# marcottelab/FluorosequencingImageAnalysis

Measured on AMD Instinct MI355X. Metric: psf_lm_fits_per_sec, higher is better.
Workload: dtype f64

## Files before the change

fluorosequencingimageanalysis_amd/csrc/fsq_fit_rounds.hip:

```cpp
#include <algorithm>
#include <atomic>
#include <cstdlib>

#include <mutex>
#include <new>
#include <type_traits>
#include <vector>

#include "fsq_common.h"
#include "fsq_lm_quad.h"
#include "fsq_evalguard.h"

namespace {

#define WAVE_SYNC() do { __builtin_amdgcn_fence(__ATOMIC_RELEASE, "wavefront"); __builtin_amdgcn_wave_barrier(); \
                         __builtin_amdgcn_fence(__ATOMIC_ACQUIRE, "wavefront"); } while (0)

#ifdef FSQ_DEBUG_HZ
__device__ unsigned long long g_hz[32];
#endif
#ifdef FSQ_PHASE_PROFILE
__device__ unsigned long long g_rphase[32];
#define RPH_DECL unsigned long long rph_t0 = clock64(), rph_acc[16] = {0,0,0,0,0,0,0,0,0,0,0,0,0,0,0,0};
#define RPH_MARK(k) { unsigned long long t_ = clock64(); rph_acc[k] += t_ - rph_t0; rph_t0 = t_; }
#define RPH_FLUSH(off) if (threadIdx.x == 0 && (blockIdx.x & 63) == 0) { for (int k_ = 0; k_ < 16; k_++) atomicAdd(&g_rphase[(off) + k_], rph_acc[k_]); }
#else
#define RPH_DECL
#define RPH_MARK(k)
#define RPH_FLUSH(off)
#endif

enum { CNT_A = 0, CNT_BLO = 1, CNT_BHI = 2, CNT_C1 = 3, CNT_C3 = 4, CNT_SET = 8 };
enum { Q_EPS = Q_WA3 };
enum { A_IDX = 0, A_X = 1, A_DIAG = 8, A_LLIM1 = 15, A_FNORM = 16, A_PAR = 17, A_DELTA = 18, A_XNORM = 19, A_ITER = 20,
       A_HDR = 21 , A_E = 21 , A_LEN = 46,
       B_GNORM = 21, B_IPVT = 22, B_QTF = 23, B_SDIAG = 30, B_R = 37, B_LEN = 65,
       C_PARL = 65, C_PARU = 66, C_FP = 67, C_LMIT = 68, C_LEN = 69 };

struct FitOut {
    double x[FSQ_NP];
    int status, niter, nfev, pad;
};
struct FitStat {
    double vmax, vmean;
};

struct Ctx {
    uint16_t* roi;
    int pix32;
    FitOut* out;
    FitStat* stat;
    long long cap;
    long long pool;
    int* err;
    int* slow_total;
    int* done;
    int tshift;
    int wave_prio;
    int force_redo;
    int force_slow_mod;
};

enum { G_KINIT_POS = 1, G_KINIT_SLOT = 2, G_KA_BLO = 3, G_KA_BHI = 4, G_KA_OVERLAP = 5, G_KA_SLOW = 6, G_KB_C1 = 7, G_KB_C3 = 8, G_KB_A = 9,
       G_KB_BLO = 10, G_KB_BHI = 11 };
FSQ_DEV long long fsq_guard(const Ctx& c, long long v, long long limit, int code)
{
    if ((unsigned long long)v < (unsigned long long)limit) return v;
    atomicMax(c.err, code);
    return 0;
}

FSQ_DEV int wave_reserve(int* counter, bool want)
{
    const unsigned long long m = __ballot(want);
    if (m == 0) return 0;
    const int lane = threadIdx.x & 63;
    const int leader = __ffsll((long long)m) - 1;
    int base = 0;
    if (lane == leader) base = atomicAdd(counter, __popcll(m));
    base = __shfl(base, leader);
    return base + __popcll(m & ((1ull << lane) - 1ull));
}

FSQ_DEV long long wave_reserve_checked(const Ctx& c, int* counter, bool want, long long limit, int code)
{
    const int at = wave_reserve(counter, want);
    return want ? fsq_guard(c, at, limit, code) : 0;
}

struct BatchArgs {
    const uint16_t* src; const int32_t* cand; int H, W; long long n; int from_image;
    int pix_fmt;
    long long base;
    int ticket;
    int no_queue;
};

FSQ_DEV void wave_mark_done(int* done, bool term, int ticket)
{
    unsigned long long m = __ballot(term);
    const int lane = threadIdx.x & 63;
    while (m) {
        const int leader = __ffsll((long long)m) - 1;
        const int t = __shfl(ticket, leader);
        const unsigned long long mm = __ballot(term && ticket == t);
        if (lane == leader) atomicAdd(done + t, __popcll(mm));
        m &= ~mm;
    }
}

#ifndef FSQ_NT
#define FSQ_NT 0
#endif
typedef unsigned fsq_u4v __attribute__((ext_vector_type(4)));
// ... 170 lines not shown
    double d = (S[0] + S[2]) + (S[1] + S[3]);
#pragma unroll
    for (int i = 16; i < 25; i++) { double v = QL(off, i); d = fsq_fma(v, v, d); }
    return d;
}

#define KA_ROWS(i) do { if (L == 8 && ((i) % 5) == 4) __builtin_amdgcn_sched_barrier(0); } while (0)
#define KA_EVAL_LOOP _Pragma("unroll EVAL_UNROLL")
#define KA_PIN(v) do { if (FAST) asm volatile("" : "+v"(v)); } while (0)
#ifdef FSQ_DEBUG_HZ
#define KA_HZ(code, cond) do { if (cond) { hz = true; if (FAST) atomicAdd(&g_hz[code], 1ull); } } while (0)
#else
#define KA_HZ(code, cond) do { if (cond) hz = true; } while (0)
#endif
template <bool FAST, int L, bool P32 = false>
__global__ void __launch_bounds__(64, (L == 8 ? 4 : 2)) kA_jacobian(Ctx c, const double* __restrict__ QA, const int* __restrict__ cntA_p,
                                                                    double* __restrict__ QB, int* __restrict__ cnt_cur,
                                                                    double* __restrict__ SQ, int* __restrict__ slow_cnt,
                                                                    int* __restrict__ next_counters)
{
    constexpr int G = 64 / L;
    constexpr int NC = 8 / L;
    constexpr int MPX = (FSQ_NPIX + L - 1) / L;
    constexpr int MREC = (A_HDR + L - 1) / L;
    constexpr bool EVAL_ALL = FAST && L == 4;
    constexpr int EVAL_UNROLL = EVAL_ALL ? MPX : 1;
    static_assert(fsq_llim(4, 0.) == FSQ_EG_MIN_SIGMA && fsq_llim(5, 0.) == FSQ_EG_MIN_SIGMA, "fsq_evalguard.h: sigma floor != the fit's lower limit");
    __shared__ double lds[Q_KA_END * G];
    const int lane = threadIdx.x, grp = lane / L, cl = lane % L, gbase = lane - cl;
    const int n7 = FSQ_NP;
    if (c.wave_prio) __builtin_amdgcn_s_setprio(3);
    const int cntA = FAST ? *cntA_p : *slow_cnt;
    if (!FAST && blockIdx.x == 0 && threadIdx.x == 0 && cntA > 0) atomicAdd(c.slow_total, cntA);
    if (FAST && blockIdx.x == 0 && threadIdx.x < CNT_SET) next_counters[threadIdx.x] = 0;
    double col[NC][FSQ_NPIX];
    RPH_DECL
    const long long cap = c.cap;
    const int stride = gridDim.x * G;
    int base = blockIdx.x * G;
    if (base >= cntA) return;
    do {
        RPH_MARK(0)
        const bool active = (base + grp) < cntA;
        const NtQ qa = ntq(QA + (active ? base + grp : 0));
        double rec[MREC];
#pragma unroll
        for (int m = 0; m < MREC; m++) { const int f = cl + L * m; rec[m] = (active && f < A_HDR) ? (double)qa[f * cap] : 0.0; }
        bool hz = false, qhz = false;
        int emin = 0;
        int tag, niter, nfev, hist;
        unpack2(__shfl(rec[A_IDX / L], gbase + A_IDX % L), &tag, &hist);
        unpack2(__shfl(rec[A_ITER / L], gbase + A_ITER % L), &niter, &nfev);
        const bool b_hi = hist > 1;
        const int at_lo = wave_reserve(cnt_cur + CNT_BLO, active && cl == 0 && !b_hi);
        const int at_hi = wave_reserve(cnt_cur + CNT_BHI, active && cl == 0 && b_hi);
#ifdef FSQ_EXPERIMENT_EXTRA_ATOMICS_KA
        {
            int sink = 0;
            for (int x = 0; x < FSQ_EXPERIMENT_EXTRA_ATOMICS_KA; x++) sink += wave_reserve(cnt_cur + 5 + (x & 1), active && cl == 0);
            if (sink == 0x7fffffff) atomicMax(c.err, 99);
        }
#endif
        if (active && cl == 0) {
            if (!b_hi) fsq_guard(c, at_lo, cap, G_KA_BLO); else fsq_guard(c, at_hi, cap, G_KA_BHI);
            if ((long long)at_lo + (long long)at_hi + 2 > cap && (at_lo > 0 || at_hi > 0)) {
                const int nlo = b_hi ? cnt_cur[CNT_BLO] : at_lo + 1, nhi = b_hi ? at_hi + 1 : cnt_cur[CNT_BHI];
                if ((long long)nlo + nhi > cap) atomicMax(c.err, (int)G_KA_OVERLAP);
            }
        }
        const long long at = __shfl((active && cl == 0) ? (int)fsq_guard(c, b_hi ? (long long)(cap - 1) - at_hi : (long long)at_lo, cap, b_hi ? G_KA_BHI : G_KA_BLO) : 0, gbase);
        const int idx = tag_slot(c, tag);
        const bool fresh = active && (nfev == 0);
        double llim1 = 0., fnorm = 0., xnorm = 0., delta = 0., par_in = 0.;
        unsigned ipvt = 0x76543210u;
        int status = 0;
        double gnorm = 0.;
        uint4 roi = make_uint4(0u, 0u, 0u, 0u);
        uint4 roi_hi = make_uint4(0u, 0u, 0u, 0u);
        double ev[MPX];
#pragma unroll
        for (int m = 0; m < MPX; m++) ev[m] = 0.0;
        if (active) {
            if (P32) {
                static_assert(!P32 || L == 4, "32-bit pixels: the four-lane Jacobian round only");
                const uint32_t* r32 = (const uint32_t*)c.roi + (size_t)idx * 32 + cl * 8;
                roi = nt_ld4(r32); roi_hi = nt_ld4(r32 + 4);
            } else if (L == 4) roi = nt_ld4(c.roi + (size_t)idx * 32 + cl * 8);
            else {
                const unsigned long long w8 = fsq_bits(nt_ld((const double*)(c.roi + (size_t)idx * 32 + cl * 4)));
                roi.x = (unsigned)w8; roi.y = (unsigned)(w8 >> 32);
            }
            if (!fresh) {
#pragma unroll
                for (int m = 0; m < MPX; m++) { const int k = cl + L * m; if (k < FSQ_NPIX) ev[m] = qa[(A_E + k) * cap]; }
            }
#pragma unroll
            for (int m = 0; m < MREC; m++) {
                const int f = cl + L * m;
                if (f >= 1 && f <= 19) QL(Q_X, f - 1) = rec[m];
            }
        }
        WAVE_SYNC();
        RPH_MARK(1)
// ... 507 lines not shown
                    while (rem >= 7 - i) { rem -= 7 - i; i++; }
                    qb[(B_R + e) * cap] = QRG(i, i + rem);
                }
                for (int k = cl; k < FSQ_NP; k += L) {
                    qb[(A_X + k) * cap] = QL(Q_X, k);
                    qb[(A_DIAG + k) * cap] = QL(Q_DIAG, k);
                    qb[(B_QTF + k) * cap] = QL(Q_QTF, k);
                    qb[(B_SDIAG + k) * cap] = 0.;
                }
                if (cl == 0) {
                    qb[A_IDX * cap] = pack2(tag, hist);
                    qb[A_LLIM1 * cap] = llim1; qb[A_FNORM * cap] = fnorm; qb[A_PAR * cap] = par_in; qb[A_DELTA * cap] = delta;
                    qb[A_XNORM * cap] = xnorm; qb[A_ITER * cap] = pack2(niter, nfev);
                    qb[B_GNORM * cap] = gnorm; qb[B_IPVT * cap] = pack2((int)ipvt, 0);
                }
            } else if (active && cl == 0) qb[A_IDX * cap] = pack2(-1, 0);
        }
        RPH_MARK(6)
        base += stride;
    } while (!FAST && base < cntA);
    RPH_FLUSH(16)
}
#undef QRG
#undef REFL
#undef KA_ROWS
#undef KA_PIN
#undef KA_EVAL_LOOP
#undef KA_HZ
#pragma pop_macro("QL")

#ifndef FSQ_KA_LANES_DEFAULT
#define FSQ_KA_LANES_DEFAULT 4
#endif
#ifndef FSQ_LMPAR_FIRST
#define FSQ_LMPAR_FIRST 5
#endif
#ifndef FSQ_LMPAR_LO
#define FSQ_LMPAR_LO 1
#endif
#ifndef FSQ_KB_WAVES
#define FSQ_KB_WAVES 2
#endif
FSQ_DEV int kb_res_slot(int i) { return i < 14 ? i : i + 7; }

template <bool FAST>
FSQ_DEV bool kb_trial_gauss(const double* p, double* myscr)
{
    bool bad = false;
    double s, c;
    fsq_sincos(FSQ_PI_180 * p[6], &s, &c);
    const double rcen_x = p[3] * c - p[2] * s;
    const double rcen_y = p[3] * s + p[2] * c;
    const FsqDivisor k4 = fsq_divisor(p[4]), k5 = fsq_divisor(p[5]);
    if (FAST)
        bad = !fsq_divisor_in_range(p[4]) || !fsq_divisor_in_range(p[5]) || !(__builtin_fabs(p[2]) <= 0x1p100) ||
              !(__builtin_fabs(p[3]) <= 0x1p100) || !fsq_evalguard_ok(c, s, rcen_x, rcen_y, p[4], p[5]);
#pragma unroll 1
    for (int xi = 0; xi < 5; xi++) {
        const double x = (double)xi;
#pragma unroll
        for (int yi = 0; yi < 5; yi++) {
            const double y = (double)yi;
            const double xp = x * c - y * s;
            const double yp = x * s + y * c;
            const double nu = rcen_x - xp, nv = rcen_y - yp;
            myscr[kb_res_slot(xi * 5 + yi) * 64] = ka_gauss<FAST>(nu, nv, k4, k5);
        }
    }
    return bad;
}

FSQ_DEV double kb_late_load(const NtRef r) { asm volatile("" ::: "memory"); return (double)r; }

struct KbLimits { int lim[4]; };
template <bool ALIASED, bool P32 = false>
__global__ void __launch_bounds__(64, FSQ_KB_WAVES) kB_step(Ctx c, const double* __restrict__ QB, const double* __restrict__ QC,
                                                  const int* __restrict__ cnt_cur,
                                                  double* __restrict__ QA_next, double* __restrict__ QB_next, double* __restrict__ QC_next,
                                                  int* __restrict__ cnt_next, KbLimits lims)
{
    __shared__ double scr[32 * 64];
    if (c.wave_prio) __builtin_amdgcn_s_setprio(3);
    const int lane = threadIdx.x;
    const long long cap = c.cap;
    double* myscr = scr + lane;
    RPH_DECL
    {
        int b = blockIdx.x, seg, cnt;
        const int n_lo = cnt_cur[CNT_BLO], n_hi = cnt_cur[CNT_BHI], n_c1 = cnt_cur[CNT_C1], n_c3 = cnt_cur[CNT_C3];
        if (b < (n_c3 + 63) / 64) { seg = 3; cnt = n_c3; }
        else if ((b -= (n_c3 + 63) / 64) < (n_hi + 63) / 64) { seg = 1; cnt = n_hi; }
        else if ((b -= (n_hi + 63) / 64) < (n_c1 + 63) / 64) { seg = 2; cnt = n_c1; }
        else if ((b -= (n_c1 + 63) / 64) < (n_lo + 63) / 64) { seg = 0; cnt = n_lo; }
        else return;
        const bool resume = seg >= 2;
        const int lm_limit = lims.lim[seg];
        const int base = b * 64;
        RPH_MARK(0)
        bool live = (base + lane) < cnt;
        const int p_in = live ? (base + lane) : base;
        const NtQ qb = ntq((resume ? QC : QB) + ((seg & 1) ? cap - 1 - p_in : p_in));
        int tag = 0, dummy, niter = 1, nfev = 1, ipvt_i = 0x76543210;
        {
            int t;
            unpack2(qb[A_IDX * cap], &t, &dummy);
            if (t == -1) live = false;
            if (live) tag = t;
        }
        QuadLm q;
        double xq[FSQ_NP];
        double llim1 = 0., fnorm = 1., par = 0., delta = 1., xnorm = 1., fnorm1;
        if (live) {
            unpack2(qb[A_ITER * cap], &niter, &nfev);
            unpack2(qb[B_IPVT * cap], &ipvt_i, &dummy);
#pragma unroll
            for (int i = 0; i < FSQ_NP; i++)
#pragma unroll
                for (int k = 0; k < FSQ_NP; k++) q.r[i][k] = (k >= i) ? (double)qb[(B_R + rpk(i, k)) * cap] : 0.0;
#pragma unroll
            for (int k = 0; k < FSQ_NP; k++) {
                q.qtf[k] = qb[(B_QTF + k) * cap]; q.dg[k] = qb[(A_DIAG + k) * cap]; q.sdiag[k] = qb[(B_SDIAG + k) * cap];
                xq[k] = qb[(A_X + k) * cap];
            }
            llim1 = qb[A_LLIM1 * cap];
            fnorm = qb[A_FNORM * cap]; par = qb[A_PAR * cap]; delta = qb[A_DELTA * cap]; xnorm = qb[A_XNORM * cap];
        } else {
            const double x0[FSQ_NP] = {100., 1000., 2.5, 2.5, 1., 1., 0.};
#pragma unroll
            for (int i = 0; i < FSQ_NP; i++)
#pragma unroll
                for (int k = 0; k < FSQ_NP; k++) q.r[i][k] = (k == i) ? 1.0 : 0.0;
#pragma unroll
            for (int k = 0; k < FSQ_NP; k++) { q.qtf[k] = 0.; q.dg[k] = 1.; q.sdiag[k] = 0.; xq[k] = x0[k]; }
        }
        const unsigned ipvt = (unsigned)ipvt_i;
#define KB_GNORM() kb_late_load(qb[B_GNORM * cap])
#pragma unroll
        for (int k = 0; k < FSQ_NP; k++) myscr[k * 64] = q.dg[k];
#pragma unroll
        for (int j = 0; j < FSQ_NP; j++) q.dgp[j] = myscr[nib_get(ipvt, j) * 64];

        RPH_MARK(1)
        int lm_hist = 0;
        {
            QuadLmparSt st;
            if (!resume) quadlm_lmpar_begin<ALIASED, 64>(q, myscr, ipvt, delta, par, st);
            else if (live) {
                int it, dm;
                unpack2(qb[C_LMIT * cap], &it, &dm);
                st.par = par; st.parl = qb[C_PARL * cap]; st.paru = qb[C_PARU * cap]; st.fp = qb[C_FP * cap];
                st.iter = it; st.done = false;
            } else { st.par = 0.; st.parl = 0.; st.paru = 0.; st.fp = 0.; st.iter = 10; st.done = true; }
            RPH_MARK(7)
            quadlm_lmpar_run<ALIASED, 64>(q, myscr, ipvt, delta, st, lm_limit);
            par = st.par;
            lm_hist = st.iter;
            {
                const bool park = live && !st.done;
                const bool to_c1 = (st.iter < lims.lim[2]);
                const int at1 = (int)wave_reserve_checked(c, cnt_next + CNT_C1, park && to_c1, cap, G_KB_C1);
                const int at3 = (int)wave_reserve_checked(c, cnt_next + CNT_C3, park && !to_c1, cap, G_KB_C3);
                if (park) {
                    const NtQ qn = ntq(QC_next + (to_c1 ? (long long)at1 : cap - 1 - at3));
                    qn[A_IDX * cap] = pack2(tag, 0);
#pragma unroll
                    for (int k = 0; k < FSQ_NP; k++) {
                        qn[(A_X + k) * cap] = xq[k]; qn[(A_DIAG + k) * cap] = q.dg[k];
                        qn[(B_QTF + k) * cap] = q.qtf[k]; qn[(B_SDIAG + k) * cap] = q.sdiag[k];
                    }
                    qn[A_LLIM1 * cap] = llim1; qn[A_FNORM * cap] = fnorm; qn[A_PAR * cap] = par; qn[A_DELTA * cap] = delta;
                    qn[A_XNORM * cap] = xnorm; qn[A_ITER * cap] = pack2(niter, nfev);
                    qn[B_GNORM * cap] = KB_GNORM(); qn[B_IPVT * cap] = pack2((int)ipvt, 0);
#pragma unroll
                    for (int i = 0; i < FSQ_NP; i++)
#pragma unroll
                        for (int k = i; k < FSQ_NP; k++) qn[(B_R + rpk(i, k)) * cap] = q.r[i][k];
                    qn[C_PARL * cap] = st.parl; qn[C_PARU * cap] = st.paru; qn[C_FP * cap] = st.fp;
                    qn[C_LMIT * cap] = pack2(st.iter, 0);
                }
                live = live && !park;
            }
        }
        RPH_MARK(2)
        double wa1[FSQ_NP], wa2[FSQ_NP];
        bool lpeg[FSQ_NP], upeg[FSQ_NP];
        int nlpeg = 0, nupeg = 0;
#pragma unroll
        for (int k = 0; k < FSQ_NP; k++) {
            wa1[k] = -q.xp[k];
            lpeg[k] = (xq[k] == fsq_llim(k, llim1)); nlpeg += lpeg[k];
            upeg[k] = fsq_qulim(k) && (xq[k] == fsq_ulim(k)); nupeg += upeg[k];
        }
// ... 133 lines not shown
            xnorm = fsq_sqrt(xs);
            fnorm = fnorm1;
            niter = niter + 1;
        }
        int status = 0;
        bool c1 = (__builtin_fabs(actred) <= 1e-10) && (prered <= 1e-10) && (0.5 * ratio <= 1);
        if (c1) status = 1;
        if (delta <= 1e-10 * xnorm) status = 2;
        if (c1 && (status == 2)) status = 3;
        if (status == 0) {
            if (niter >= 200) status = 5;
            if ((__builtin_fabs(actred) <= FSQ_MACHEP) && (prered <= FSQ_MACHEP) && (0.5 * ratio <= 1)) status = 6;
            if (delta <= FSQ_MACHEP * xnorm) status = 7;
            if (KB_GNORM() <= FSQ_MACHEP) status = 8;
        }
        if (status == 0 && !accepted) {
            bool fin = __builtin_isfinite(ratio);
#pragma unroll
            for (int k = 0; k < FSQ_NP; k++)
                fin = fin && __builtin_isfinite(wa1[k]) && __builtin_isfinite(wa2[k]) && __builtin_isfinite(xq[k]);
            if (!fin) status = -16;
        }
        RPH_MARK(5)
        if (live && status != 0) {
            FitOut o;
#pragma unroll
            for (int k = 0; k < FSQ_NP; k++) o.x[k] = xq[k];
            o.status = status; o.niter = niter; o.nfev = nfev; o.pad = 0;
            c.out[tag_slot(c, tag)] = o;
        }
        wave_mark_done(c.done, live && status != 0, tag_ticket(c, tag));
        {
            const bool toA = live && status == 0 && accepted, toB = live && status == 0 && !accepted;
            const bool hi = lm_hist > 1;
#ifdef FSQ_EXPERIMENT_EXTRA_ATOMICS_KB
            {
                int sink = 0;
                for (int x = 0; x < FSQ_EXPERIMENT_EXTRA_ATOMICS_KB; x++) sink += wave_reserve(cnt_next + 5 + (x & 1), live);
                if (sink == 0x7fffffff) atomicMax(c.err, 99);
            }
#endif
            const int atA = (int)wave_reserve_checked(c, cnt_next + CNT_A, toA, cap, G_KB_A);
            const int atBl = (int)wave_reserve_checked(c, cnt_next + CNT_BLO, toB && !hi, cap, G_KB_BLO);
            const int atBh = (int)wave_reserve_checked(c, cnt_next + CNT_BHI, toB && hi, cap, G_KB_BHI);
            if (toA || toB) {
                const NtQ qn = ntq(toA ? (QA_next + atA) : (QB_next + (hi ? cap - 1 - atBh : (long long)atBl)));
                qn[A_IDX * cap] = pack2(tag, lm_hist);
#pragma unroll
                for (int k = 0; k < FSQ_NP; k++) { qn[(A_X + k) * cap] = xq[k]; qn[(A_DIAG + k) * cap] = q.dg[k]; }
                qn[A_LLIM1 * cap] = llim1; qn[A_FNORM * cap] = fnorm; qn[A_PAR * cap] = par; qn[A_DELTA * cap] = delta;
                qn[A_XNORM * cap] = xnorm; qn[A_ITER * cap] = pack2(niter, nfev);
                if (toA) {
#pragma unroll
                    for (int i = 0; i < FSQ_NPIX; i++) qn[(A_E + i) * cap] = myscr[kb_res_slot(i) * 64];
                }
                if (toB) {
                    qn[B_GNORM * cap] = KB_GNORM(); qn[B_IPVT * cap] = pack2((int)ipvt, 0);
#pragma unroll
                    for (int k = 0; k < FSQ_NP; k++) { qn[(B_QTF + k) * cap] = q.qtf[k]; qn[(B_SDIAG + k) * cap] = q.sdiag[k]; }
#undef KB_GNORM
#pragma unroll
                    for (int i = 0; i < FSQ_NP; i++)
#pragma unroll
                        for (int k = i; k < FSQ_NP; k++) qn[(B_R + rpk(i, k)) * cap] = q.r[i][k];
                }
            }
        }
        RPH_MARK(6)
    }
    RPH_FLUSH(0)
}

__global__ void __launch_bounds__(64) kfinish(Ctx c, BatchArgs b, FsqRow* __restrict__ rows)
{
    long long i = (long long)blockIdx.x * blockDim.x + threadIdx.x;
    if (i >= b.n) return;
    const long long slot = b.base + i;
    const FitOut S = c.out[slot];
    double data[FSQ_NPIX], p[FSQ_NP];
// ... 177 lines not shown
    (void)hipFree(d_bad);
    *mismatches = (int64_t)h;
    return FSQ_OK;
}

extern "C" int64_t fsq_fit_last_slow_count(void) { return g_last_slow.load(); }
#ifdef FSQ_DEBUG_HZ
extern "C" int fsq_debug_hz(unsigned long long* out32, int reset)
{
    FSQ_HIP_CHECK(hipDeviceSynchronize());
    FSQ_HIP_CHECK(hipMemcpyFromSymbol(out32, HIP_SYMBOL(g_hz), sizeof(unsigned long long) * 32));
    if (reset) { unsigned long long z[32] = {0}; FSQ_HIP_CHECK(hipMemcpyToSymbol(HIP_SYMBOL(g_hz), z, sizeof(z))); }
    return FSQ_OK;
}
#endif

#ifdef FSQ_PHASE_PROFILE
extern "C" int fsq_debug_rphase(unsigned long long* out32, int reset)
{
    unsigned long long* p = nullptr;
    if (hipGetSymbolAddress((void**)&p, HIP_SYMBOL(g_rphase)) != hipSuccess) return -1;
    if (hipMemcpy(out32, p, 32 * 8, hipMemcpyDeviceToHost) != hipSuccess) return -1;
    if (reset) (void)hipMemset(p, 0, 32 * 8);
    return 0;
}
#endif

static size_t al256(size_t v) { return (v + 255) & ~(size_t)255; }

namespace {
enum { CTL_SLOW_TOTAL = 2 * CNT_SET, CTL_SLOW_CNT = 2 * CNT_SET + 1, CTL_F32_NEXT = 2 * CNT_SET + 2, CTL_ERR = 2 * CNT_SET + 3, CTL_DONE = 2 * CNT_SET + 8, CTL_INTS = CTL_DONE + FSQ_MAX_TICKETS };

struct RoundsCfg {
    int lm_first = FSQ_LMPAR_FIRST, lm_lo = FSQ_LMPAR_LO, sync_mask = 3, force_slow_mod = 0, force_redo = 0, no_wave_prio = 0, trace = 0;
    int ka_lanes = FSQ_KA_LANES_DEFAULT;
    int max_rounds = 0, ka_lds_pad = 0, kb_lds_pad = 0;
    long long two_pass_min = 524288, hiprio_below = 200000;
};
RoundsCfg read_cfg()
{
    RoundsCfg g;
    const char* e;
    if ((e = getenv("FSQ_DEBUG_FORCE_SLOW")) != nullptr) g.force_slow_mod = atoi(e);
    if ((e = getenv("FSQ_DEBUG_FORCE_NORM_RECOMPUTE")) != nullptr) g.force_redo = atoi(e) ? 1 : 0;
    if ((e = getenv("FSQ_LMPAR_FIRST_ITERS")) != nullptr && atoi(e) >= 1 && atoi(e) <= 10) g.lm_first = atoi(e);
    if ((e = getenv("FSQ_LMPAR_LO_ITERS")) != nullptr && atoi(e) >= 1 && atoi(e) <= 10) g.lm_lo = atoi(e);
    if ((e = getenv("FSQ_TWO_PASS_MIN")) != nullptr) g.two_pass_min = atoll(e);
    if ((e = getenv("FSQ_HIPRIO_BELOW")) != nullptr) g.hiprio_below = atoll(e);
    if ((e = getenv("FSQ_SYNC_EVERY")) != nullptr && atoi(e) >= 1) g.sync_mask = atoi(e) - 1;
    if (getenv("FSQ_NO_WAVE_PRIO")) g.no_wave_prio = 1;
    if (getenv("FSQ_DEBUG_TRACE")) g.trace = 1;
    if ((e = getenv("FSQ_DEBUG_MAX_ROUNDS")) != nullptr) g.max_rounds = atoi(e);
    if ((e = getenv("FSQ_KA_LANES")) != nullptr && (atoi(e) == 4 || atoi(e) == 8)) g.ka_lanes = atoi(e);
    if ((e = getenv("FSQ_DEBUG_KA_LDS_PAD")) != nullptr) g.ka_lds_pad = atoi(e);
    if ((e = getenv("FSQ_DEBUG_KB_LDS_PAD")) != nullptr) g.kb_lds_pad = atoi(e);
    return g;
}

struct HiStream { hipStream_t s; int dev; bool busy; };
std::mutex g_hi_mu;
std::vector<HiStream> g_hi;
hipStream_t hi_acquire()
{
    int dev = 0;
    if (hipGetDevice(&dev) != hipSuccess) return nullptr;
    std::lock_guard<std::mutex> lk(g_hi_mu);
    for (auto& h : g_hi)
        if (!h.busy && h.dev == dev) { h.busy = true; return h.s; }
    int least = 0, greatest = 0;
    if (hipDeviceGetStreamPriorityRange(&least, &greatest) != hipSuccess) return nullptr;
    hipStream_t st = nullptr;
    if (hipStreamCreateWithPriority(&st, hipStreamNonBlocking, greatest) != hipSuccess) return nullptr;
    g_hi.push_back({st, dev, true});
    return st;
}
void hi_release(hipStream_t st)
{
    std::lock_guard<std::mutex> lk(g_hi_mu);
    for (auto& h : g_hi)
        if (h.s == st) h.busy = false;
}

enum { FSQ_TICKET_BITS = 5 };
static_assert((1 << FSQ_TICKET_BITS) == FSQ_MAX_TICKETS, "ticket bits");
enum { T_FREE = 0, T_FLIGHT = 1, T_FINISHED = 2 };
struct Batch { BatchArgs a; FsqRow* rows; int state; hipEvent_t ev; };

size_t cap_round(size_t q) { return (q + 255) & ~(size_t)255; }

size_t layout_bytes(size_t pool, size_t qcap)
{
    qcap = cap_round(qcap);
    size_t b = 4096;
    b += al256(pool * 128) + al256(pool * sizeof(FitOut)) + al256(pool * sizeof(FitStat));
    b += 2 * al256(qcap * A_LEN * 8) + 2 * al256(qcap * B_LEN * 8) + 2 * al256(qcap * C_LEN * 8) + al256(qcap * A_LEN * 8);
    return b;
}
}

struct FsqFitQueue {
    Ctx c;
    size_t pool = 0, qcap = 0;
    int* ctl = nullptr;
    double *QA[2], *QB[2], *QC[2], *SQ = nullptr;
    int *cset[2], *cSlow = nullptr;
    RoundsCfg cfg;
    bool ref = true, f32 = false, single_call = false;
    int cus = 256;
    long long round = 0;
    long long boundA = 0, alive = 0, slow_pending = 0;
    long long head = 0;
    Batch b[FSQ_MAX_TICKETS];
    hipStream_t s = nullptr, s_finish = nullptr, hi = nullptr;
    int h_ctl[CTL_INTS];
    void* owned_ws = nullptr;

    int init(void* d_ws, int64_t ws_bytes, size_t pool_, size_t qcap_, int mode, hipStream_t stream, bool single)
    {
        if (!d_ws || (size_t)ws_bytes < layout_bytes(pool_, qcap_)) return FSQ_ENOMEM;
        qcap_ = cap_round(qcap_);
        if (pool_ > 2000000000ull || qcap_ > 2000000000ull) return FSQ_ENOTIMPL;
        pool = pool_; qcap = qcap_; s = s_finish = stream; single_call = single;
        ref = ((mode & 0xff) == FSQ_MODE_REF);
        f32 = ((mode & 0xff) == FSQ_MODE_TEXTBOOK_F32);
        cfg = read_cfg();
        unsigned char* ws = (unsigned char*)d_ws;
        ctl = (int*)ws;
        size_t o = 4096;
        c.cap = (long long)qcap;
        c.roi = (uint16_t*)(ws + o); o += al256(pool * 128);
        c.pix32 = (mode & FSQ_PIXELS_U32_FLAG) ? 1 : 0;
        c.out = (FitOut*)(ws + o); o += al256(pool * sizeof(FitOut));
        c.stat = (FitStat*)(ws + o); o += al256(pool * sizeof(FitStat));
        QA[0] = (double*)(ws + o); o += al256(qcap * A_LEN * 8);
        QA[1] = (double*)(ws + o); o += al256(qcap * A_LEN * 8);
        QB[0] = (double*)(ws + o); o += al256(qcap * B_LEN * 8);
        QB[1] = (double*)(ws + o); o += al256(qcap * B_LEN * 8);
        QC[0] = (double*)(ws + o); o += al256(qcap * C_LEN * 8);
        QC[1] = (double*)(ws + o); o += al256(qcap * C_LEN * 8);
        SQ = (double*)(ws + o); o += al256(qcap * A_LEN * 8);
        cset[0] = ctl; cset[1] = ctl + CNT_SET;
        cSlow = ctl + CTL_SLOW_CNT;
        c.slow_total = ctl + CTL_SLOW_TOTAL; c.done = ctl + CTL_DONE; c.err = ctl + CTL_ERR; c.pool = (long long)pool;
        c.tshift = single ? 31 : 32 - FSQ_TICKET_BITS;
        if (!single && pool_ >= (1ull << c.tshift)) return FSQ_ENOTIMPL;
        c.wave_prio = 0; c.force_redo = cfg.force_redo; c.force_slow_mod = cfg.force_slow_mod;
        int dev = 0;
        if (hipGetDevice(&dev) == hipSuccess) (void)hipDeviceGetAttribute(&cus, hipDeviceAttributeMultiprocessorCount, dev);
        for (auto& t : b) { t.state = T_FREE; t.ev = nullptr; t.rows = nullptr; }
        FSQ_HIP_CHECK(hipMemsetAsync(ctl, 0, CTL_INTS * sizeof(int), s));
        return FSQ_OK;
    }

    long long alloc_slots(long long n)
    {
        if ((size_t)n > pool) return -1;
        long long at = head;
        for (int attempt = 0; attempt < 2; attempt++) {
            if ((size_t)(at + n) > pool) at = 0;
            bool clash = false;
            for (const auto& t : b)
                if (t.state == T_FLIGHT && at < t.a.base + t.a.n && t.a.base < at + n) { clash = true; break; }
            if (!clash) { head = at + n; return at; }
            if (at == 0) break;
            at = 0;
        }
        return -1;
    }

    int submit(const uint16_t* src, int pix_fmt, int H, int W, const int32_t* cand, long long n, bool from_image, FsqRow* rows, int* ticket)
// ... 24 lines not shown
            hipLaunchKernelGGL(kfinish, dim3((unsigned)((n + 63) / 64)), dim3(64), 0, s, c, B.a, rows);
            if (B.ev) FSQ_HIP_CHECK(hipEventRecord(B.ev, s));
            B.state = T_FINISHED;
        } else {
            const int cur = (int)(round & 1);
            FSQ_HIP_CHECK(hipMemsetAsync(c.done + t, 0, sizeof(int), s));
            hipLaunchKernelGGL(kinit, dim3((unsigned)((n + 255) / 256)), dim3(256), 0, s, c, B.a, QA[cur], cset[cur] + CNT_A);
            B.state = T_FLIGHT;
            boundA += n; alive += n;
        }
        if (ticket) *ticket = t;
        return FSQ_OK;
    }

    int one_round()
    {
        const int cur = (int)(round & 1), nxt = cur ^ 1;
        const int G = 64 / cfg.ka_lanes;
        const long long gA = (boundA + G - 1) / G;
        if (slow_pending > 0) {
            if (c.pix32) hipLaunchKernelGGL((kA_jacobian<false, 4, true>), dim3((unsigned)std::min<long long>((alive + 15) / 16, (long long)cus * 8)), dim3(64), 0, s, c, SQ, cSlow, QB[cur], cset[cur], SQ, cSlow, cset[nxt]);
            else hipLaunchKernelGGL((kA_jacobian<false, 4>), dim3((unsigned)std::min<long long>((alive + 15) / 16, (long long)cus * 8)), dim3(64), 0, s, c, SQ, cSlow, QB[cur], cset[cur], SQ, cSlow, cset[nxt]);
            FSQ_HIP_CHECK(hipMemsetAsync(cSlow, 0, sizeof(int), s));
            slow_pending = 0;
        }
        if (gA > 0 && c.pix32)
            hipLaunchKernelGGL((kA_jacobian<true, 4, true>), dim3((unsigned)gA), dim3(64), cfg.ka_lds_pad, s, c, QA[cur], cset[cur] + CNT_A, QB[cur], cset[cur], SQ, cSlow, cset[nxt]);
        else if (gA > 0 && cfg.ka_lanes == 8)
            hipLaunchKernelGGL((kA_jacobian<true, 8>), dim3((unsigned)gA), dim3(64), cfg.ka_lds_pad, s, c, QA[cur], cset[cur] + CNT_A, QB[cur], cset[cur], SQ, cSlow, cset[nxt]);
        else if (gA > 0)
            hipLaunchKernelGGL((kA_jacobian<true, 4>), dim3((unsigned)gA), dim3(64), cfg.ka_lds_pad, s, c, QA[cur], cset[cur] + CNT_A, QB[cur], cset[cur], SQ, cSlow, cset[nxt]);
        else
            FSQ_HIP_CHECK(hipMemsetAsync(cset[nxt], 0, CNT_SET * sizeof(int), s));
        const long long gB = (alive + 63) / 64 + 4;
        {
            const bool staged = alive > cfg.two_pass_min && cfg.lm_first < 10;
            KbLimits lims;
            lims.lim[0] = staged ? std::min(cfg.lm_lo, cfg.lm_first) : 10; lims.lim[1] = staged ? cfg.lm_first : 10; lims.lim[2] = staged ? cfg.lm_first : 10; lims.lim[3] = 10;
            if (c.pix32 && ref) hipLaunchKernelGGL((kB_step<true, true>), dim3((unsigned)gB), dim3(64), 0, s, c, QB[cur], QC[cur], cset[cur], QA[nxt], QB[nxt], QC[nxt], cset[nxt], lims);
            else if (c.pix32) hipLaunchKernelGGL((kB_step<false, true>), dim3((unsigned)gB), dim3(64), 0, s, c, QB[cur], QC[cur], cset[cur], QA[nxt], QB[nxt], QC[nxt], cset[nxt], lims);
            else if (ref) hipLaunchKernelGGL((kB_step<true>), dim3((unsigned)gB), dim3(64), cfg.kb_lds_pad, s, c, QB[cur], QC[cur], cset[cur], QA[nxt], QB[nxt], QC[nxt], cset[nxt], lims);
            else hipLaunchKernelGGL((kB_step<false>), dim3((unsigned)gB), dim3(64), 0, s, c, QB[cur], QC[cur], cset[cur], QA[nxt], QB[nxt], QC[nxt], cset[nxt], lims);
        }
        boundA = alive;
        round++;
        return FSQ_OK;
    }

    int look(int* newly_finished)
    {
        FSQ_HIP_CHECK(hipMemcpyAsync(h_ctl, ctl, sizeof(h_ctl), hipMemcpyDeviceToHost, s));
        FSQ_HIP_CHECK(hipStreamSynchronize(s));
        const int cur = (int)(round & 1);
        const int* hc = h_ctl + CNT_SET * cur;
        boundA = hc[CNT_A];
        slow_pending = h_ctl[CTL_SLOW_CNT];
        alive = boundA + hc[CNT_BLO] + hc[CNT_BHI] + hc[CNT_C1] + hc[CNT_C3] + slow_pending;
        g_last_slow.store(h_ctl[CTL_SLOW_TOTAL]);
        if (h_ctl[CTL_ERR] != 0) {
            fprintf(stderr, "fsq: fit queue invariant %d broken (cap %lld, pool %lld, host bounds: A %lld alive %lld; counters A %d B %d+%d C %d+%d slow %d)\n",
                    h_ctl[CTL_ERR], (long long)qcap, (long long)pool, boundA, alive, hc[CNT_A], hc[CNT_BLO], hc[CNT_BHI], hc[CNT_C1], hc[CNT_C3], h_ctl[CTL_SLOW_CNT]);
            return FSQ_EINTERNAL;
        }
        if (cfg.trace) fprintf(stderr, "round %lld: A=%lld B=%d+%d C=%d+%d slow=%lld total_slow=%d\n", round - 1, boundA, hc[CNT_BLO], hc[CNT_BHI], hc[CNT_C1], hc[CNT_C3], slow_pending, h_ctl[CTL_SLOW_TOTAL]);
        int fin = 0;
        for (auto& t : b) {
            if (t.state != T_FLIGHT || h_ctl[CTL_DONE + t.a.ticket] < t.a.n) continue;
            hipLaunchKernelGGL(kfinish, dim3((unsigned)((t.a.n + 63) / 64)), dim3(64), 0, s_finish, c, t.a, t.rows);
            if (t.ev) FSQ_HIP_CHECK(hipEventRecord(t.ev, s_finish));
            t.state = T_FINISHED;
            fin++;
        }
        if (newly_finished) *newly_finished = fin;
        if (single_call && !hi && alive > 0 && alive < cfg.hiprio_below && (long long)pool >= 4 * cfg.hiprio_below) {
            hi = hi_acquire();
            if (hi) s = hi;
            c.wave_prio = cfg.no_wave_prio ? 0 : 1;
        }
        return FSQ_OK;
    }

    int advance(long long max_rounds, long long alive_below, long long* alive_out, int* finished_out)
    {
        int fin_total = 0;
        long long ran = 0;
        while (alive > 0) {
            int rc = one_round();
            if (rc != FSQ_OK) return rc;
            ran++;
            const bool stop = (max_rounds > 0 && ran >= max_rounds);
            if (stop || (round & cfg.sync_mask) == 0) {
                int fin = 0;
                rc = look(&fin);
                if (rc != FSQ_OK) return rc;
                fin_total += fin;
                if (stop || fin_total > 0 || alive < alive_below) break;
            }
// ... 117 lines not shown
```

Baseline: 22.93 million.

## Split LM step queue into four history-based lists with per-list lmpar iteration limits

```diff
diff --git a/fluorosequencingimageanalysis_amd/csrc/fsq_fit_rounds.hip b/fluorosequencingimageanalysis_amd/csrc/fsq_fit_rounds.hip
--- a/fluorosequencingimageanalysis_amd/csrc/fsq_fit_rounds.hip
+++ b/fluorosequencingimageanalysis_amd/csrc/fsq_fit_rounds.hip
@@ -10,6 +10,7 @@
 #include "fsq_common.h"
 #include "fsq_lm_quad.h"
 #include "fsq_evalguard.h"
+#include "fsq_kb_tilemap.h"
 
 namespace {
 
@@ -30,7 +31,9 @@
 #define RPH_FLUSH(off)
 #endif
 
-enum { CNT_A = 0, CNT_BLO = 1, CNT_BHI = 2, CNT_C1 = 3, CNT_C3 = 4, CNT_SET = 8 };
+enum { CNT_LINE = 32, CNT_A = 0, CNT_B0 = CNT_LINE, CNT_C1 = CNT_B0 + KB_C1 * CNT_LINE, CNT_C3 = CNT_B0 + KB_C3 * CNT_LINE,
+       CNT_KINDS = 1 + KB_LISTS, CNT_SET = 8 * CNT_LINE };
+__host__ __device__ inline int cnt_of_list(int list) { return CNT_B0 + list * CNT_LINE; }
 enum { Q_EPS = Q_WA3 };
 enum { A_IDX = 0, A_X = 1, A_DIAG = 8, A_LLIM1 = 15, A_FNORM = 16, A_PAR = 17, A_DELTA = 18, A_XNORM = 19, A_ITER = 20,
        A_HDR = 21 , A_E = 21 , A_LEN = 46,
@@ -61,8 +64,8 @@
     int force_slow_mod;
 };
 
-enum { G_KINIT_POS = 1, G_KINIT_SLOT = 2, G_KA_BLO = 3, G_KA_BHI = 4, G_KA_OVERLAP = 5, G_KA_SLOW = 6, G_KB_C1 = 7, G_KB_C3 = 8, G_KB_A = 9,
-       G_KB_BLO = 10, G_KB_BHI = 11 };
+enum { G_KINIT_POS = 1, G_KINIT_SLOT = 2, G_KA_B = 3, G_KA_OVERLAP = 5, G_KA_SLOW = 6, G_KB_C1 = 7, G_KB_C3 = 8, G_KB_A = 9,
+       G_KB_B = 10 };
 FSQ_DEV long long fsq_guard(const Ctx& c, long long v, long long limit, int code)
 {
     if ((unsigned long long)v < (unsigned long long)limit) return v;
@@ -80,6 +83,23 @@
     if (lane == leader) base = atomicAdd(counter, __popcll(m));
     base = __shfl(base, leader);
     return base + __popcll(m & ((1ull << lane) - 1ull));
+}
+
+FSQ_DEV int wave_reserve4(int* counters, bool want, int list, int* other)
+{
+    const int lane = threadIdx.x & 63;
+    unsigned long long m[4];
+#pragma unroll
+    for (int l = 0; l < 4; l++) m[l] = __ballot(want && list == l);
+    const unsigned long long mine = list == 0 ? m[0] : list == 1 ? m[1] : list == 2 ? m[2] : m[3];
+    const unsigned long long pair = list == 0 ? m[1] : list == 1 ? m[0] : list == 2 ? m[3] : m[2];
+    const int leader = want ? __ffsll((long long)mine) - 1 : lane;
+    int base = 0;
+    if (want && lane == leader) base = atomicAdd(counters + list * CNT_LINE, __popcll(mine));
+    const int pair_base = __shfl(base, pair ? __ffsll((long long)pair) - 1 : lane);
+    base = __shfl(base, leader);
+    *other = pair ? pair_base + __popcll(pair) : 0;
+    return want ? base + __popcll(mine & ((1ull << lane) - 1ull)) : 0;
 }
 
 FSQ_DEV long long wave_reserve_checked(const Ctx& c, int* counter, bool want, long long limit, int code)
@@ -316,7 +336,7 @@
     if (c.wave_prio) __builtin_amdgcn_s_setprio(3);
     const int cntA = FAST ? *cntA_p : *slow_cnt;
     if (!FAST && blockIdx.x == 0 && threadIdx.x == 0 && cntA > 0) atomicAdd(c.slow_total, cntA);
-    if (FAST && blockIdx.x == 0 && threadIdx.x < CNT_SET) next_counters[threadIdx.x] = 0;
+    if (FAST && blockIdx.x == 0 && threadIdx.x < CNT_KINDS) next_counters[threadIdx.x * CNT_LINE] = 0;
     double col[NC][FSQ_NPIX];
     RPH_DECL
     const long long cap = c.cap;
@@ -335,24 +355,16 @@
         int tag, niter, nfev, hist;
         unpack2(__shfl(rec[A_IDX / L], gbase + A_IDX % L), &tag, &hist);
         unpack2(__shfl(rec[A_ITER / L], gbase + A_ITER % L), &niter, &nfev);
-        const bool b_hi = hist > 1;
-        const int at_lo = wave_reserve(cnt_cur + CNT_BLO, active && cl == 0 && !b_hi);
-        const int at_hi = wave_reserve(cnt_cur + CNT_BHI, active && cl == 0 && b_hi);
-#ifdef FSQ_EXPERIMENT_EXTRA_ATOMICS_KA
-        {
-            int sink = 0;
-            for (int x = 0; x < FSQ_EXPERIMENT_EXTRA_ATOMICS_KA; x++) sink += wave_reserve(cnt_cur + 5 + (x & 1), active && cl == 0);
-            if (sink == 0x7fffffff) atomicMax(c.err, 99);
-        }
-#endif
+        const int blist = kb_list_of_history(hist);
+        int at_pair;
+        const int at_mine = wave_reserve4(cnt_cur + CNT_B0, active && cl == 0, blist, &at_pair);
         if (active && cl == 0) {
-            if (!b_hi) fsq_guard(c, at_lo, cap, G_KA_BLO); else fsq_guard(c, at_hi, cap, G_KA_BHI);
-            if ((long long)at_lo + (long long)at_hi + 2 > cap && (at_lo > 0 || at_hi > 0)) {
-                const int nlo = b_hi ? cnt_cur[CNT_BLO] : at_lo + 1, nhi = b_hi ? at_hi + 1 : cnt_cur[CNT_BHI];
-                if ((long long)nlo + nhi > cap) atomicMax(c.err, (int)G_KA_OVERLAP);
-            }
-        }
-        const long long at = __shfl((active && cl == 0) ? (int)fsq_guard(c, b_hi ? (long long)(cap - 1) - at_hi : (long long)at_lo, cap, b_hi ? G_KA_BHI : G_KA_BLO) : 0, gbase);
+            if ((long long)at_mine + (long long)at_pair + 2 > cap && (at_mine > 0 || at_pair > 0)) {
+                if ((long long)at_mine + 1 + cnt_cur[cnt_of_list(blist ^ 1)] > cap) atomicMax(c.err, (int)G_KA_OVERLAP);
+            }
+        }
+        const long long at = __shfl((active && cl == 0) ? (int)kb_list_pos(blist, fsq_guard(c, at_mine, cap, G_KA_B), cap) : 0, gbase)
+                             + (long long)kb_list_array(blist) * (B_LEN * cap);
         const int idx = tag_slot(c, tag);
         const bool fresh = active && (nfev == 0);
         double llim1 = 0., fnorm = 0., xnorm = 0., delta = 0., par_in = 0.;
@@ -926,11 +938,8 @@
 #ifndef FSQ_KA_LANES_DEFAULT
 #define FSQ_KA_LANES_DEFAULT 4
 #endif
-#ifndef FSQ_LMPAR_FIRST
-#define FSQ_LMPAR_FIRST 5
-#endif
-#ifndef FSQ_LMPAR_LO
-#define FSQ_LMPAR_LO 1
+#ifndef FSQ_LMPAR_LIMITS
+#define FSQ_LMPAR_LIMITS {0, 3, 3, 10, 3, 10}
 #endif
 #ifndef FSQ_KB_WAVES
 #define FSQ_KB_WAVES 2
@@ -966,7 +975,7 @@
 
 FSQ_DEV double kb_late_load(const NtRef r) { asm volatile("" ::: "memory"); return (double)r; }
 
-struct KbLimits { int lim[4]; };
+struct KbLimits { int lim[KB_LISTS]; };
 template <bool ALIASED, bool P32 = false>
 __global__ void __launch_bounds__(64, FSQ_KB_WAVES) kB_step(Ctx c, const double* __restrict__ QB, const double* __restrict__ QC,
                                                   const int* __restrict__ cnt_cur,
@@ -980,20 +989,19 @@
     double* myscr = scr + lane;
     RPH_DECL
     {
-        int b = blockIdx.x, seg, cnt;
-        const int n_lo = cnt_cur[CNT_BLO], n_hi = cnt_cur[CNT_BHI], n_c1 = cnt_cur[CNT_C1], n_c3 = cnt_cur[CNT_C3];
-        if (b < (n_c3 + 63) / 64) { seg = 3; cnt = n_c3; }
-        else if ((b -= (n_c3 + 63) / 64) < (n_hi + 63) / 64) { seg = 1; cnt = n_hi; }
-        else if ((b -= (n_hi + 63) / 64) < (n_c1 + 63) / 64) { seg = 2; cnt = n_c1; }
-        else if ((b -= (n_c1 + 63) / 64) < (n_lo + 63) / 64) { seg = 0; cnt = n_lo; }
-        else return;
-        const bool resume = seg >= 2;
+        int n_in[KB_LISTS];
+#pragma unroll
+        for (int l = 0; l < KB_LISTS; l++) n_in[l] = cnt_cur[cnt_of_list(l)];
+        const KbTile tile = kb_tile_of_block(blockIdx.x, n_in);
+        if (tile.list < 0) return;
+        const int seg = tile.list, cnt = tile.count;
+        const bool resume = seg >= KB_C1;
         const int lm_limit = lims.lim[seg];
-        const int base = b * 64;
+        const int base = tile.tile * 64;
         RPH_MARK(0)
         bool live = (base + lane) < cnt;
         const int p_in = live ? (base + lane) : base;
-        const NtQ qb = ntq((resume ? QC : QB) + ((seg & 1) ? cap - 1 - p_in : p_in));
+        const NtQ qb = ntq((resume ? QC : QB + (long long)kb_list_array(seg) * (B_LEN * cap)) + kb_list_pos(seg, p_in, cap));
         int tag = 0, dummy, niter = 1, nfev = 1, ipvt_i = 0x76543210;
         {
             int t;
@@ -1051,7 +1059,7 @@
             lm_hist = st.iter;
             {
                 const bool park = live && !st.done;
-                const bool to_c1 = (st.iter < lims.lim[2]);
+                const bool to_c1 = (st.iter < lims.lim[KB_C1]);
                 const int at1 = (int)wave_reserve_checked(c, cnt_next + CNT_C1, park && to_c1, cap, G_KB_C1);
                 const int at3 = (int)wave_reserve_checked(c, cnt_next + CNT_C3, park && !to_c1, cap, G_KB_C3);
                 if (park) {
@@ -1251,19 +1259,13 @@
         wave_mark_done(c.done, live && status != 0, tag_ticket(c, tag));
         {
             const bool toA = live && status == 0 && accepted, toB = live && status == 0 && !accepted;
-            const bool hi = lm_hist > 1;
-#ifdef FSQ_EXPERIMENT_EXTRA_ATOMICS_KB
-            {
-                int sink = 0;
-                for (int x = 0; x < FSQ_EXPERIMENT_EXTRA_ATOMICS_KB; x++) sink += wave_reserve(cnt_next + 5 + (x & 1), live);
-                if (sink == 0x7fffffff) atomicMax(c.err, 99);
-            }
-#endif
+            const int blist = kb_list_of_history(lm_hist);
             const int atA = (int)wave_reserve_checked(c, cnt_next + CNT_A, toA, cap, G_KB_A);
-            const int atBl = (int)wave_reserve_checked(c, cnt_next + CNT_BLO, toB && !hi, cap, G_KB_BLO);
-            const int atBh = (int)wave_reserve_checked(c, cnt_next + CNT_BHI, toB && hi, cap, G_KB_BHI);
+            int atB_pair;
+            const int atB = wave_reserve4(cnt_next + CNT_B0, toB, blist, &atB_pair);
             if (toA || toB) {
-                const NtQ qn = ntq(toA ? (QA_next + atA) : (QB_next + (hi ? cap - 1 - atBh : (long long)atBl)));
+                const NtQ qn = ntq(toA ? (QA_next + atA)
+                                       : (QB_next + (long long)kb_list_array(blist) * (B_LEN * cap) + kb_list_pos(blist, fsq_guard(c, atB, cap, G_KB_B), cap)));
                 qn[A_IDX * cap] = pack2(tag, lm_hist);
 #pragma unroll
                 for (int k = 0; k < FSQ_NP; k++) { qn[(A_X + k) * cap] = xq[k]; qn[(A_DIAG + k) * cap] = q.dg[k]; }
@@ -1507,7 +1509,8 @@
 enum { CTL_SLOW_TOTAL = 2 * CNT_SET, CTL_SLOW_CNT = 2 * CNT_SET + 1, CTL_F32_NEXT = 2 * CNT_SET + 2, CTL_ERR = 2 * CNT_SET + 3, CTL_DONE = 2 * CNT_SET + 8, CTL_INTS = CTL_DONE + FSQ_MAX_TICKETS };
 
 struct RoundsCfg {
-    int lm_first = FSQ_LMPAR_FIRST, lm_lo = FSQ_LMPAR_LO, sync_mask = 3, force_slow_mod = 0, force_redo = 0, no_wave_prio = 0, trace = 0;
+    int lm_lim[KB_LISTS] = FSQ_LMPAR_LIMITS;
+    int sync_mask = 3, force_slow_mod = 0, force_redo = 0, no_wave_prio = 0, trace = 0;
     int ka_lanes = FSQ_KA_LANES_DEFAULT;
     int max_rounds = 0, ka_lds_pad = 0, kb_lds_pad = 0;
     long long two_pass_min = 524288, hiprio_below = 200000;
@@ -1518,8 +1521,13 @@
     const char* e;
     if ((e = getenv("FSQ_DEBUG_FORCE_SLOW")) != nullptr) g.force_slow_mod = atoi(e);
     if ((e = getenv("FSQ_DEBUG_FORCE_NORM_RECOMPUTE")) != nullptr) g.force_redo = atoi(e) ? 1 : 0;
-    if ((e = getenv("FSQ_LMPAR_FIRST_ITERS")) != nullptr && atoi(e) >= 1 && atoi(e) <= 10) g.lm_first = atoi(e);
-    if ((e = getenv("FSQ_LMPAR_LO_ITERS")) != nullptr && atoi(e) >= 1 && atoi(e) <= 10) g.lm_lo = atoi(e);
+    if ((e = getenv("FSQ_LMPAR_FIRST_ITERS")) != nullptr && atoi(e) >= 1 && atoi(e) <= 10) g.lm_lim[KB_B3] = g.lm_lim[KB_C1] = atoi(e);
+    if ((e = getenv("FSQ_LMPAR_LO_ITERS")) != nullptr && atoi(e) >= 1 && atoi(e) <= 10) g.lm_lim[KB_B1] = atoi(e);
+    if ((e = getenv("FSQ_LMPAR_B0_ITERS")) != nullptr && atoi(e) >= 0 && atoi(e) <= 10) g.lm_lim[KB_B0] = atoi(e);
+    if ((e = getenv("FSQ_LMPAR_B1_ITERS")) != nullptr && atoi(e) >= 0 && atoi(e) <= 10) g.lm_lim[KB_B1] = atoi(e);
+    if ((e = getenv("FSQ_LMPAR_B3_ITERS")) != nullptr && atoi(e) >= 0 && atoi(e) <= 10) g.lm_lim[KB_B3] = atoi(e);
+    if ((e = getenv("FSQ_LMPAR_B10_ITERS")) != nullptr && atoi(e) >= 0 && atoi(e) <= 10) g.lm_lim[KB_B10] = atoi(e);
+    if ((e = getenv("FSQ_LMPAR_C1_ITERS")) != nullptr && atoi(e) >= 1 && atoi(e) <= 10) g.lm_lim[KB_C1] = atoi(e);
     if ((e = getenv("FSQ_TWO_PASS_MIN")) != nullptr) g.two_pass_min = atoll(e);
     if ((e = getenv("FSQ_HIPRIO_BELOW")) != nullptr) g.hiprio_below = atoll(e);
     if ((e = getenv("FSQ_SYNC_EVERY")) != nullptr && atoi(e) >= 1) g.sync_mask = atoi(e) - 1;
@@ -1568,7 +1576,7 @@
     qcap = cap_round(qcap);
     size_t b = 4096;
     b += al256(pool * 128) + al256(pool * sizeof(FitOut)) + al256(pool * sizeof(FitStat));
-    b += 2 * al256(qcap * A_LEN * 8) + 2 * al256(qcap * B_LEN * 8) + 2 * al256(qcap * C_LEN * 8) + al256(qcap * A_LEN * 8);
+    b += 2 * al256(qcap * A_LEN * 8) + 2 * al256(2 * qcap * B_LEN * 8) + 2 * al256(qcap * C_LEN * 8) + al256(qcap * A_LEN * 8);
     return b;
 }
 }
@@ -1609,8 +1617,8 @@
         c.stat = (FitStat*)(ws + o); o += al256(pool * sizeof(FitStat));
         QA[0] = (double*)(ws + o); o += al256(qcap * A_LEN * 8);
         QA[1] = (double*)(ws + o); o += al256(qcap * A_LEN * 8);
-        QB[0] = (double*)(ws + o); o += al256(qcap * B_LEN * 8);
-        QB[1] = (double*)(ws + o); o += al256(qcap * B_LEN * 8);
+        QB[0] = (double*)(ws + o); o += al256(2 * qcap * B_LEN * 8);
+        QB[1] = (double*)(ws + o); o += al256(2 * qcap * B_LEN * 8);
         QC[0] = (double*)(ws + o); o += al256(qcap * C_LEN * 8);
         QC[1] = (double*)(ws + o); o += al256(qcap * C_LEN * 8);
         SQ = (double*)(ws + o); o += al256(qcap * A_LEN * 8);
@@ -1701,11 +1709,12 @@
             hipLaunchKernelGGL((kA_jacobian<true, 4>), dim3((unsigned)gA), dim3(64), cfg.ka_lds_pad, s, c, QA[cur], cset[cur] + CNT_A, QB[cur], cset[cur], SQ, cSlow, cset[nxt]);
         else
             FSQ_HIP_CHECK(hipMemsetAsync(cset[nxt], 0, CNT_SET * sizeof(int), s));
-        const long long gB = (alive + 63) / 64 + 4;
+        const long long gB = kb_grid_for(alive);
         {
-            const bool staged = alive > cfg.two_pass_min && cfg.lm_first < 10;
+            const bool staged = alive > cfg.two_pass_min;
             KbLimits lims;
-            lims.lim[0] = staged ? std::min(cfg.lm_lo, cfg.lm_first) : 10; lims.lim[1] = staged ? cfg.lm_first : 10; lims.lim[2] = staged ? cfg.lm_first : 10; lims.lim[3] = 10;
+            for (int l = 0; l < KB_LISTS; l++) lims.lim[l] = staged ? cfg.lm_lim[l] : 10;
+            lims.lim[KB_C3] = 10;
             if (c.pix32 && ref) hipLaunchKernelGGL((kB_step<true, true>), dim3((unsigned)gB), dim3(64), 0, s, c, QB[cur], QC[cur], cset[cur], QA[nxt], QB[nxt], QC[nxt], cset[nxt], lims);
             else if (c.pix32) hipLaunchKernelGGL((kB_step<false, true>), dim3((unsigned)gB), dim3(64), 0, s, c, QB[cur], QC[cur], cset[cur], QA[nxt], QB[nxt], QC[nxt], cset[nxt], lims);
             else if (ref) hipLaunchKernelGGL((kB_step<true>), dim3((unsigned)gB), dim3(64), cfg.kb_lds_pad, s, c, QB[cur], QC[cur], cset[cur], QA[nxt], QB[nxt], QC[nxt], cset[nxt], lims);
@@ -1724,14 +1733,22 @@
         const int* hc = h_ctl + CNT_SET * cur;
         boundA = hc[CNT_A];
         slow_pending = h_ctl[CTL_SLOW_CNT];
-        alive = boundA + hc[CNT_BLO] + hc[CNT_BHI] + hc[CNT_C1] + hc[CNT_C3] + slow_pending;
+        int nl[KB_LISTS];
+        for (int l = 0; l < KB_LISTS; l++) nl[l] = hc[cnt_of_list(l)];
+        alive = boundA + slow_pending;
+        for (int l = 0; l < KB_LISTS; l++) alive += nl[l];
         g_last_slow.store(h_ctl[CTL_SLOW_TOTAL]);
         if (h_ctl[CTL_ERR] != 0) {
-            fprintf(stderr, "fsq: fit queue invariant %d broken (cap %lld, pool %lld, host bounds: A %lld alive %lld; counters A %d B %d+%d C %d+%d slow %d)\n",
-                    h_ctl[CTL_ERR], (long long)qcap, (long long)pool, boundA, alive, hc[CNT_A], hc[CNT_BLO], hc[CNT_BHI], hc[CNT_C1], hc[CNT_C3], h_ctl[CTL_SLOW_CNT]);
+            fprintf(stderr, "fsq: fit queue invariant %d broken (cap %lld, pool %lld, host bounds: A %lld alive %lld; counters A %d B %d+%d+%d+%d C %d+%d slow %d)\n",
+                    h_ctl[CTL_ERR], (long long)qcap, (long long)pool, boundA, alive, hc[CNT_A], nl[KB_B0], nl[KB_B1], nl[KB_B3], nl[KB_B10], nl[KB_C1], nl[KB_C3], h_ctl[CTL_SLOW_CNT]);
             return FSQ_EINTERNAL;
         }
-        if (cfg.trace) fprintf(stderr, "round %lld: A=%lld B=%d+%d C=%d+%d slow=%lld total_slow=%d\n", round - 1, boundA, hc[CNT_BLO], hc[CNT_BHI], hc[CNT_C1], hc[CNT_C3], slow_pending, h_ctl[CTL_SLOW_TOTAL]);
+        if (cfg.trace) {
+            const int* hp = h_ctl + CNT_SET * (cur ^ 1);
+            fprintf(stderr, "round %lld: left A=%lld B=%d+%d+%d+%d C=%d+%d slow=%lld total_slow=%d stepped B=%d+%d+%d+%d C=%d+%d\n", round - 1, boundA,
+                    nl[KB_B0], nl[KB_B1], nl[KB_B3], nl[KB_B10], nl[KB_C1], nl[KB_C3], slow_pending, h_ctl[CTL_SLOW_TOTAL],
+                    hp[cnt_of_list(KB_B0)], hp[cnt_of_list(KB_B1)], hp[cnt_of_list(KB_B3)], hp[cnt_of_list(KB_B10)], hp[cnt_of_list(KB_C1)], hp[cnt_of_list(KB_C3)]);
+        }
         int fin = 0;
         for (auto& t : b) {
             if (t.state != T_FLIGHT || h_ctl[CTL_DONE + t.a.ticket] < t.a.n) continue;
diff --git a/fluorosequencingimageanalysis_amd/csrc/fsq_kb_tilemap.h b/fluorosequencingimageanalysis_amd/csrc/fsq_kb_tilemap.h
--- /dev/null
+++ b/fluorosequencingimageanalysis_amd/csrc/fsq_kb_tilemap.h
@@ -0,0 +1,39 @@
+#pragma once
+
+#if defined(__HIPCC__) || defined(__CUDACC__)
+#define FSQ_KB_FN __host__ __device__ inline
+#else
+#define FSQ_KB_FN inline
+#endif
+
+enum { KB_B0 = 0, KB_B1 = 1, KB_B3 = 2, KB_B10 = 3, KB_C1 = 4, KB_C3 = 5, KB_LISTS = 6 };
+enum { KB_TILE = 64 };
+
+FSQ_KB_FN int kb_list_of_history(int hist) { return hist <= 0 ? KB_B0 : hist == 1 ? KB_B1 : hist <= 4 ? KB_B3 : KB_B10; }
+FSQ_KB_FN int kb_list_array(int list) { return list == KB_B3 || list == KB_B10; }
+FSQ_KB_FN bool kb_list_down(int list) { return (list & 1) != 0; }
+FSQ_KB_FN long long kb_list_pos(int list, long long p, long long cap) { return kb_list_down(list) ? cap - 1 - p : p; }
+
+FSQ_KB_FN int kb_tiles(int n) { return n / KB_TILE + (n % KB_TILE != 0); }
+
+FSQ_KB_FN int kb_launch_order(int k)
+{
+    return k == 0 ? KB_C3 : k == 1 ? KB_B10 : k == 2 ? KB_C1 : k == 3 ? KB_B3 : k == 4 ? KB_B1 : KB_B0;
+}
+
+struct KbTile { int list, tile, count; };
+
+FSQ_KB_FN KbTile kb_tile_of_block(long long block, const int* n)
+{
+    KbTile t; t.list = -1; t.tile = 0; t.count = 0;
+    if (block < 0) return t;
+    for (int k = 0; k < KB_LISTS; k++) {
+        const int l = kb_launch_order(k);
+        const int tiles = n[l] > 0 ? kb_tiles(n[l]) : 0;
+        if (block < tiles) { t.list = l; t.tile = (int)block; t.count = n[l]; return t; }
+        block -= tiles;
+    }
+    return t;
+}
+
+FSQ_KB_FN long long kb_grid_for(long long alive) { return alive / KB_TILE + (alive % KB_TILE != 0) + KB_LISTS; }
```

Measured after the change: 23.46 million (median of 6 runs). +2.3%, better.
